# xeTaiz/vit-tf

Measured on AMD Instinct MI355X. Metric: slices/sec (ViT-S/8, 512^3 vol: feature volume + 16-query similarity), higher is better.
Workload: dtype fp16; 1 GPU; 512^3 CT-like synthetic volume (seed 0), ViT-S/8, fos 64: 1536 slices of 512x512 (N=4097) per step + 16-query similarity -> the metric's configuration (BASELINE configs[2]); engine_batch=512, weights=seeded synthetic vits8 (seed 0), parallelism=single GPU

## Files before the change

### vit-tf_amd/csrc/attention_pp64.hip

```cpp
#include "attn_common.h"

#include <stdlib.h>

namespace {

constexpr int NBUF = 3;
constexpr int QT = 256;
constexpr int KT = ATT_KT;
constexpr int KVB = ATT_KV_TILE_BYTES;
constexpr int BUFB = ATT_BUF_BYTES;

struct LdsBases { const char *ka0, *ka1, *ka2, *ka3, *va0, *va1; };
struct KFrag { s16x8_t k[4]; };
struct VFrag { s16x8_t v[4]; };
struct QFrag { s16x8_t q[4]; };
struct Blk {
  f32x16_t o0, o1, negm;
  float l_run;
};

__device__ __forceinline__ s16x8_t ld_k(const LdsBases& b, int i, int off) {
  const char* base = i == 0 ? b.ka0 : i == 1 ? b.ka1 : i == 2 ? b.ka2 : b.ka3;
  return *reinterpret_cast<const s16x8_t*>(base + off);
}
__device__ __forceinline__ s16x8_t ld_v(const LdsBases& b, int j, int off) {
  const int imm = off + 2048 * (j >> 1) + 512 * (j & 1);
  const s16x4_t lo = __builtin_amdgcn_ds_read_tr16_b64_v4i16((__attribute__((address_space(3))) s16x4_t*)(b.va0 + imm));
  const s16x4_t hi = __builtin_amdgcn_ds_read_tr16_b64_v4i16((__attribute__((address_space(3))) s16x4_t*)(b.va1 + imm + 1024));
  return __builtin_shufflevector(lo, hi, 0, 1, 2, 3, 4, 5, 6, 7);
}

template <int DT> __device__ __forceinline__ f32x16_t score_mfma(const KFrag& k, const QFrag& q, f32x16_t c) {
#pragma unroll
  for (int i = 0; i < 4; ++i) c = mfma32<DT>(k.k[i], q.q[i], c);
  return c;
}

__device__ __forceinline__ float tile_max(const f32x16_t& s) {
  float tmax = max3_f32(s[0], s[1], s[2]);
#pragma unroll
  for (int r = 3; r < 15; r += 2) tmax = max3_f32(tmax, s[r], s[r + 1]);
  tmax = fmaxf(tmax, s[15]);
  const unsigned tb = __float_as_uint(tmax);
  const auto sw = __builtin_amdgcn_permlane32_swap(tb, tb, false, false);
  return max3_f32(tmax, __uint_as_float(sw[0]), __uint_as_float(sw[1]));
}

__device__ unsigned g_rescales;

template <int DT> __device__ __forceinline__ constexpr float p_limit() { return DT == VITTF_FP16 ? 8192.f : 1073741824.f; }

template <int DT>
__device__ __forceinline__ float rescale_block(const LdsBases& b, Blk& X, const QFrag& qX, s16x8_t (&pX)[2], int ck_off, bool mask,
                                               int key0, int tokens, int h) {
  if ((threadIdx.x & 63) == 0) atomicAdd(&g_rescales, 1u);
  f32x16_t raw;
#pragma unroll
  for (int r = 0; r < 16; ++r) raw[r] = 0.f;
  KFrag kh;
#pragma unroll
  for (int i = 0; i < 4; ++i) kh.k[i] = ld_k(b, i, ck_off);
  raw = score_mfma<DT>(kh, qX, raw);
  if (mask) {
#pragma unroll
    for (int r = 0; r < 16; ++r)
      if (key0 + acc_row(r, h) >= tokens) raw[r] = -INFINITY;
  }
  const float tmax = tile_max(raw);
  const float delta = fmaxf(tmax + X.negm[0], 0.f);
  const float alpha = __builtin_amdgcn_exp2f(-delta);
  X.l_run *= alpha;
#pragma unroll
  for (int r = 0; r < 16; ++r) {
    X.o0[r] *= alpha;
    X.o1[r] *= alpha;
    X.negm[r] -= delta;
  }
  float psum0 = 0.f, psum1 = 0.f;
  u32x4_t u0, u1;
#pragma unroll
  for (int i = 0; i < 8; ++i) {
    const float e0 = __builtin_amdgcn_exp2f(raw[2 * i] + X.negm[2 * i]);
    const float e1 = __builtin_amdgcn_exp2f(raw[2 * i + 1] + X.negm[2 * i + 1]);
    psum0 += e0;
    psum1 += e1;
    const unsigned w = pack2_h16<DT>(e0, e1);
    if (i < 4) u0[i] = w; else u1[i - 4] = w;
  }
  pX[0] = __builtin_bit_cast(s16x8_t, u0);
  pX[1] = __builtin_bit_cast(s16x8_t, u1);
  return psum0 + psum1;
}

template <int DT, bool LOAD, bool MASK>
__device__ __forceinline__ void pp_phase(const LdsBases& b, Blk& X, const QFrag& qX, f32x16_t& sX, s16x8_t (&pX)[2], Blk& Y,
                                         const QFrag& qY, f32x16_t& sY, const s16x8_t (&pY)[2], KFrag& kf, VFrag& vf, int ck_off,
                                         int nk_off, int nv_off, int key0, int tokens, int h) {
  if constexpr (MASK) {
#pragma unroll
    for (int r = 0; r < 16; ++r)
      if (key0 + acc_row(r, h) >= tokens) sX[r] = -INFINITY;
  }
  float psum0 = 0.f, psum1 = 0.f;
  u32x4_t pk0, pk1;
#pragma unroll
  for (int g = 0; g < 8; ++g) {
    const int i = g & 3;
    if (g < 4) {
      sY = mfma32<DT>(kf.k[i], qY.q[i], i == 0 ? Y.negm : sY);
      if constexpr (LOAD) kf.k[i] = ld_k(b, i, nk_off);
    } else {
      if (i & 1) Y.o1 = mfma32<DT>(vf.v[i], pY[i >> 1], Y.o1);
      else       Y.o0 = mfma32<DT>(vf.v[i], pY[i >> 1], Y.o0);
      if constexpr (LOAD) vf.v[i] = ld_v(b, i, nv_off);
    }
    const float e0 = __builtin_amdgcn_exp2f(sX[2 * g]);
    const float e1 = __builtin_amdgcn_exp2f(sX[2 * g + 1]);
    if (g == 0) { psum0 = e0; psum1 = e1; } else { psum0 += e0; psum1 += e1; }
    const unsigned w = pack2_h16<DT>(e0, e1);
    if (g < 4) pk0[g] = w; else pk1[g - 4] = w;
    __builtin_amdgcn_sched_barrier(0);
  }
  float ps = psum0 + psum1;
  pX[0] = __builtin_bit_cast(s16x8_t, pk0);
  pX[1] = __builtin_bit_cast(s16x8_t, pk1);
  if (__builtin_expect(__any(!(ps <= p_limit<DT>())), 0)) ps = rescale_block<DT>(b, X, qX, pX, ck_off, MASK, key0, tokens, h);
  X.l_run += ps;
}

template <int DT>
__device__ __forceinline__ void pp_phase_rt(const LdsBases& b, Blk& X, const QFrag& qX, f32x16_t& sX, s16x8_t (&pX)[2], Blk& Y,
                                            const QFrag& qY, f32x16_t& sY, const s16x8_t (&pY)[2], KFrag& kf, VFrag& vf,
                                            int ck_off, int nk_off, int nv_off, bool do_s, bool do_o, bool load_k, bool load_v,
                                            bool mask, int key0, int tokens, int h) {
  if (do_s) sY = score_mfma<DT>(kf, qY, Y.negm);
  if (do_o) {
#pragma unroll
    for (int j = 0; j < 4; ++j) {
      if (j & 1) Y.o1 = mfma32<DT>(vf.v[j], pY[j >> 1], Y.o1);
      else       Y.o0 = mfma32<DT>(vf.v[j], pY[j >> 1], Y.o0);
    }
  }
  if (load_k) {
#pragma unroll
    for (int i = 0; i < 4; ++i) kf.k[i] = ld_k(b, i, nk_off);
  }
  if (load_v) {
#pragma unroll
    for (int j = 0; j < 4; ++j) vf.v[j] = ld_v(b, j, nv_off);
  }
  if (mask) {
#pragma unroll
    for (int r = 0; r < 16; ++r)
      if (key0 + acc_row(r, h) >= tokens) sX[r] = -INFINITY;
  }
  float psum0 = 0.f, psum1 = 0.f;
  u32x4_t pk0, pk1;
#pragma unroll
  for (int g = 0; g < 8; ++g) {
    const float e0 = __builtin_amdgcn_exp2f(sX[2 * g]);
    const float e1 = __builtin_amdgcn_exp2f(sX[2 * g + 1]);
    psum0 += e0;
    psum1 += e1;
    const unsigned w = pack2_h16<DT>(e0, e1);
    if (g < 4) pk0[g] = w; else pk1[g - 4] = w;
  }
  float ps = psum0 + psum1;
  pX[0] = __builtin_bit_cast(s16x8_t, pk0);
  pX[1] = __builtin_bit_cast(s16x8_t, pk1);
  if (__builtin_expect(__any(!(ps <= p_limit<DT>())), 0)) ps = rescale_block<DT>(b, X, qX, pX, ck_off, mask, key0, tokens, h);
  X.l_run += ps;
}

template <int DT>
__global__ __launch_bounds__(256, 2) void attn_pp64_kernel(const unsigned short* __restrict__ qkv, unsigned short* __restrict__ out,
                                                           int tokens, int heads, int q_tiles, int total) {
  __shared__ __attribute__((aligned(16))) char smem[NBUF * BUFB];
  const int tid = threadIdx.x;
  const int lane = tid & 63, wave = tid >> 6;
  const int h = lane >> 5, l31 = lane & 31;

  const int item = xcd_remap(blockIdx.x, total);
  const int qt = item % q_tiles;
  const int bh = item / q_tiles;
  const int hd = bh % heads, bi = bh / heads;
  const int dmodel = heads * 64;
  const int ld = 3 * dmodel;
  const unsigned short* base = qkv + (int64_t)bi * tokens * ld;

  const i32x4_t rsrc = lds_dma_rsrc(base, (unsigned)((int64_t)tokens * ld * 2));

  QFrag qa, qb;
  const int qrow_a = qt * QT + wave * 64 + l31, qrow_b = qrow_a + 32;
  {
    const unsigned short* pa_ = base + (int64_t)(qrow_a < tokens ? qrow_a : tokens - 1) * ld + hd * 64 + 8 * h;
    const unsigned short* pb_ = base + (int64_t)(qrow_b < tokens ? qrow_b : tokens - 1) * ld + hd * 64 + 8 * h;
#pragma unroll
    for (int i = 0; i < 4; ++i) {
      qa.q[i] = *reinterpret_cast<const s16x8_t*>(pa_ + 16 * i);
      qb.q[i] = *reinterpret_cast<const s16x8_t*>(pb_ + 16 * i);
    }
  }

  int voff_k, voff_v;
  {
    int r, cc, key, ch;
    tile_pos(tid, r, cc);
    voff_k = (r * ld + dmodel + hd * 64 + cc * 8) * 2;
    v_pos(tid, key, ch);
    voff_v = (key * ld + 2 * dmodel + hd * 64 + ch * 8) * 2;
  }
  const int tile_stride = KT * ld * 2, half_stride = 32 * ld * 2;
  const int nt = (tokens + KT - 1) / KT;
  const unsigned dma_dst = (unsigned)(size_t)LDS_PTR(smem) + (__builtin_amdgcn_readfirstlane(tid & ~63) << 4);
#define PP_STAGE_TILE(t_, bufi_)                                                                    \
  {                                                                                                 \
    const int so_ = (t_) * tile_stride;                                                             \
    const unsigned dst_ = dma_dst + (bufi_) * BUFB;                                                 \
    if ((t_) == nt - 1) {                                                                           \
      int vk_ = voff_k, vv_ = voff_v;    \
      asm volatile("" : "+v"(vk_), "+v"(vv_));                                                      \
      _Pragma("unroll") for (int i_ = 0; i_ < 2; ++i_) {                                            \
        lds_dma16(rsrc, dst_ + i_ * 4096, vk_ + so_ + i_ * half_stride, 0);                         \
        lds_dma16(rsrc, dst_ + KVB + i_ * 4096, vv_ + so_ + i_ * half_stride, 0);                   \
      }                                                                                             \
    } else {                                                                                        \
      _Pragma("unroll") for (int i_ = 0; i_ < 2; ++i_) {                                            \
        lds_dma16(rsrc, dst_ + i_ * 4096, voff_k, so_ + i_ * half_stride);                          \
        lds_dma16(rsrc, dst_ + KVB + i_ * 4096, voff_v, so_ + i_ * half_stride);                    \
      }                                                                                             \
    }                                                                                               \
  }

  LdsBases b;
  {
    const int p_l = l31 >> 1;
    const int bslot = (((l31 & 1) << 3) | h) ^ (p_l & 15);
    b.ka0 = smem + (p_l << 8) + ((bslot ^ 0) << 4);
    b.ka1 = smem + (p_l << 8) + ((bslot ^ 2) << 4);
    b.ka2 = smem + (p_l << 8) + ((bslot ^ 4) << 4);
    b.ka3 = smem + (p_l << 8) + ((bslot ^ 6) << 4);
    const int g16 = lane >> 4;
    const int tr_q = (lane & 15) >> 2;
    const int tr_p = lane & 3;
    const int tr_ch = 2 * (g16 & 1) + (tr_p >> 1);
    const int vl0 = 64 * (4 * h + tr_q) + 16 * (tr_ch ^ h) + 8 * (tr_p & 1);
    b.va0 = smem + vl0;
    b.va1 = smem + (vl0 ^ 32);
  }

  PP_STAGE_TILE(0, 0)
  if (nt > 1) PP_STAGE_TILE(1, 1)
  asm volatile("s_waitcnt vmcnt(0)" ::: "memory");
  __syncthreads();
  if (nt > 2) PP_STAGE_TILE(2, 2)
  asm volatile("" : "+v"(qa.q[0]), "+v"(qa.q[1]), "+v"(qa.q[2]), "+v"(qa.q[3]), "+v"(qb.q[0]), "+v"(qb.q[1]), "+v"(qb.q[2]), "+v"(qb.q[3]));

#define PP_TILE_BARRIER(BNEXT2)                                                                     \
  {                                                                                                 \
    asm volatile("s_waitcnt vmcnt(0)" ::: "memory");                                                \
    __syncthreads();                                                                                \
    if (t + 2 < nt) PP_STAGE_TILE(t + 2, BNEXT2)                                                    \
  }

  const bool active = __builtin_amdgcn_readfirstlane(qt * QT + wave * 64) < tokens;
  if (!active) {
    for (int t = 1; t < nt; ++t) {
      const int b2 = (t + 2) % NBUF;
      PP_TILE_BARRIER(b2)
    }
    return;
  }

  Blk A, B;
  f32x16_t sa, sb;
  s16x8_t pa[2], pb[2];
  KFrag kf;
  VFrag vf = {};
#pragma unroll
  for (int r = 0; r < 16; ++r) { A.o0[r] = 0.f; A.o1[r] = 0.f; A.negm[r] = 0.f; B.o0[r] = 0.f; B.o1[r] = 0.f; B.negm[r] = 0.f; }
  A.l_run = 0.f; B.l_run = 0.f;
  pa[0] = s16x8_t{}; pa[1] = s16x8_t{}; pb[0] = s16x8_t{}; pb[1] = s16x8_t{};
  {
#pragma unroll
    for (int i = 0; i < 4; ++i) kf.k[i] = ld_k(b, i, 0);
    sa = score_mfma<DT>(kf, qa, A.negm);
    sb = score_mfma<DT>(kf, qb, B.negm);
    if (nt == 1) {
#pragma unroll
      for (int r = 0; r < 16; ++r)
        if (acc_row(r, h) >= tokens) { sa[r] = -INFINITY; sb[r] = -INFINITY; }
    }
    const float ta = tile_max(sa), tb = tile_max(sb);
#pragma unroll
    for (int r = 0; r < 16; ++r) { A.negm[r] = -ta; sa[r] -= ta; B.negm[r] = -tb; sb[r] -= tb; }
  }

#define PP_TILE(RB_)                                                                                                        \
  {                                                                                                                         \
    constexpr int o_ = (RB_) * BUFB, on_ = (((RB_) + 1) % NBUF) * BUFB;                                                     \
    pp_phase<DT, true, false>(b, A, qa, sa, pa, B, qb, sb, pb, kf, vf, o_, o_ + 4096, o_ + KVB, 0, tokens, h);              \
    pp_phase<DT, false, false>(b, B, qb, sb, pb, A, qa, sa, pa, kf, vf, o_, 0, 0, 0, tokens, h);                            \
    pp_phase<DT, true, false>(b, A, qa, sa, pa, B, qb, sb, pb, kf, vf, o_ + 4096, on_, o_ + KVB + 4096, 0, tokens, h);      \
    pp_phase<DT, false, false>(b, B, qb, sb, pb, A, qa, sa, pa, kf, vf, o_ + 4096, 0, 0, 0, tokens, h);                     \
    ++t;                                                                                                                    \
  }
#define PP_COLD_TILE()                                                                                                      \
  {                                                                                                                         \
    const int o_ = (t % NBUF) * BUFB, on_ = ((t + 1) % NBUF) * BUFB;                                                        \
    const bool first_ = t == 0, last_ = t == nt - 1;                                                                        \
                      \
    const bool half_ = last_ && tokens - t * KT <= 32;                                                                      \
    int hc_ = h;             \
    asm volatile("" : "+v"(hc_));                                                                                           \
    pp_phase_rt<DT>(b, A, qa, sa, pa, B, qb, sb, pb, kf, vf, o_, o_ + 4096, o_ + KVB, !first_, !first_, !half_, true, last_, \
                    t * KT, tokens, hc_);                                                                                     \
    pp_phase_rt<DT>(b, B, qb, sb, pb, A, qa, sa, pa, kf, vf, o_, 0, 0, !half_, true, false, false, last_, t * KT, tokens, hc_); \
    if (!half_) {                                                                                                           \
      pp_phase_rt<DT>(b, A, qa, sa, pa, B, qb, sb, pb, kf, vf, o_ + 4096, on_, o_ + KVB + 4096, true, true, !last_, true,    \
                      last_, t * KT + 32, tokens, hc_);                                                                       \
      pp_phase_rt<DT>(b, B, qb, sb, pb, A, qa, sa, pa, kf, vf, o_ + 4096, 0, 0, !last_, true, false, false, last_,           \
                      t * KT + 32, tokens, hc_);                                                                              \
    }                                                                                                                       \
    ++t;                                                                                                                    \
  }
  int t = 0;
  PP_COLD_TILE()
  while (t + 3 <= nt - 1) {
    PP_TILE_BARRIER(0) PP_TILE(1)
    PP_TILE_BARRIER(1) PP_TILE(2)
    PP_TILE_BARRIER(2) PP_TILE(0)
  }
  while (t < nt) {
    const int b2_ = (t + 2) % NBUF;
    PP_TILE_BARRIER(b2_)
    PP_COLD_TILE()
  }
#undef PP_COLD_TILE
#undef PP_TILE
#undef PP_TILE_BARRIER
#undef PP_STAGE_TILE
#pragma unroll
  for (int j = 0; j < 4; ++j) {
    if (j & 1) B.o1 = mfma32<DT>(vf.v[j], pb[j >> 1], B.o1);
    else       B.o0 = mfma32<DT>(vf.v[j], pb[j >> 1], B.o0);
  }

  auto store = [&](const Blk& X, int qrow) {
    const unsigned lb = __float_as_uint(X.l_run);
    const auto sw = __builtin_amdgcn_permlane32_swap(lb, lb, false, false);
    const float inv = 1.0f / (__uint_as_float(sw[0]) + __uint_as_float(sw[1]));
    if (qrow < tokens) store_o_row<DT>(out + ((int64_t)bi * tokens + qrow) * dmodel + hd * 64, h, X.o0, X.o1, inv);
  };
  store(A, qrow_a);
  store(B, qrow_b);
}

}

extern "C" int64_t vittf_attention_rescale_count(int32_t reset) {
  unsigned v = 0;
  if (hipDeviceSynchronize() != hipSuccess) return VITTF_ERR_LAUNCH;
  if (hipMemcpyFromSymbol(&v, HIP_SYMBOL(g_rescales), sizeof(v)) != hipSuccess) return VITTF_ERR_LAUNCH;
  if (reset) {
    const unsigned z = 0;
    if (hipMemcpyToSymbol(HIP_SYMBOL(g_rescales), &z, sizeof(z)) != hipSuccess) return VITTF_ERR_LAUNCH;
  }
  return (int64_t)v;
}

int vittf_attention_pp64(const void* qkv, void* out, int32_t batch, int32_t tokens, int32_t heads, int32_t dtype, hipStream_t st) {
  const int q_tiles = (tokens + QT - 1) / QT;
  const int64_t total64 = (int64_t)batch * heads * q_tiles;
  if (total64 > (1 << 30)) return VITTF_ERR_INVALID_ARG;
  const int total = (int)total64;
  if (dtype == VITTF_BF16)
    hipLaunchKernelGGL((attn_pp64_kernel<VITTF_BF16>), dim3(total), dim3(256), 0, st, (const unsigned short*)qkv,
                       (unsigned short*)out, tokens, heads, q_tiles, total);
  else if (dtype == VITTF_FP16)
    hipLaunchKernelGGL((attn_pp64_kernel<VITTF_FP16>), dim3(total), dim3(256), 0, st, (const unsigned short*)qkv,
                       (unsigned short*)out, tokens, heads, q_tiles, total);
  else
    return VITTF_ERR_INVALID_ARG;
  return vittf_check_launch();
}
```

Before: 2374 slices/s.

## Fold CLS key into registers and add split-key path for ragged query tile

When the token count is 64k+1 (a CLS token plus a full patch grid), the CLS key/value is loaded into registers and folded into the softmax with dot2 instructions. The remaining keys then tile exactly, so the padded, masked final KV tile goes away. The last query tile, which holds at most 32 rows, gets a dedicated path: two waves split the keys between them and merge their partial softmax states through LDS, while the other two waves act as DMA producers. This adds code size and complexity, and a noinline call that may raise register pressure.

```diff
diff --git a/vit-tf_amd/csrc/attention_pp64.hip b/vit-tf_amd/csrc/attention_pp64.hip
--- a/vit-tf_amd/csrc/attention_pp64.hip
+++ b/vit-tf_amd/csrc/attention_pp64.hip
@@ -172,6 +172,218 @@
   X.l_run += ps;
 }
 
+
+struct ClsKV { s16x8_t k[4]; s16x8_t v[2]; };
+template <int DT> __device__ __forceinline__ ClsKV load_cls_kv(const unsigned short* base, int dmodel, int hd, int h, int l31) {
+  ClsKV c;
+  const unsigned short* pk_ = base + dmodel + hd * 64 + 8 * h;
+  const unsigned short* pv_ = base + 2 * dmodel + hd * 64 + l31;
+#pragma unroll
+  for (int i = 0; i < 4; ++i) c.k[i] = *reinterpret_cast<const s16x8_t*>(pk_ + 16 * i);
+#pragma unroll
+  for (int dv = 0; dv < 2; ++dv) {
+    c.v[dv] = s16x8_t{};
+    c.v[dv][0] = h == 0 ? (short)pv_[32 * dv] : (short)0;
+  }
+  return c;
+}
+template <int DT> __device__ __forceinline__ float dot2_h16(unsigned a, unsigned b, float c) {
+  if constexpr (DT == VITTF_BF16) return __builtin_amdgcn_fdot2_f32_bf16(__builtin_bit_cast(bf16x2_t, a), __builtin_bit_cast(bf16x2_t, b), c, false);
+  else return __builtin_amdgcn_fdot2(__builtin_bit_cast(f16x2_t, a), __builtin_bit_cast(f16x2_t, b), c, false);
+}
+template <int DT> __device__ __forceinline__ void cls_fold(const ClsKV& c, const QFrag& q, int h, float& tmax, Blk& X) {
+  typedef __attribute__((ext_vector_type(4))) unsigned u4_t;
+  float s0 = 0.f, s1 = 0.f;
+#pragma unroll
+  for (int i = 0; i < 4; ++i) {
+    const u4_t qu = __builtin_bit_cast(u4_t, q.q[i]), ku = __builtin_bit_cast(u4_t, c.k[i]);
+    s0 = dot2_h16<DT>(qu[0], ku[0], s0);
+    s1 = dot2_h16<DT>(qu[1], ku[1], s1);
+    s0 = dot2_h16<DT>(qu[2], ku[2], s0);
+    s1 = dot2_h16<DT>(qu[3], ku[3], s1);
+  }
+  const unsigned sb_ = __float_as_uint(s0 + s1);
+  const auto sw = __builtin_amdgcn_permlane32_swap(sb_, sb_, false, false);
+  const float sc = __uint_as_float(sw[0]) + __uint_as_float(sw[1]);
+  tmax = fmaxf(tmax, sc);
+  const float pc = __builtin_amdgcn_exp2f(sc - tmax);
+  X.l_run = h == 0 ? pc : 0.f;
+  u4_t pu = {0u, 0u, 0u, 0u};
+  pu[0] = h == 0 ? pack2_h16<DT>(pc, 0.f) : 0u;
+  const s16x8_t pf = __builtin_bit_cast(s16x8_t, pu);
+  X.o0 = mfma32<DT>(c.v[0], pf, X.o0);
+  X.o1 = mfma32<DT>(c.v[1], pf, X.o1);
+}
+
+struct RagCtx {
+  const unsigned short* base; unsigned short* orow;
+  int tokens, heads, hd, q0; unsigned lds0;
+};
+__device__ __forceinline__ unsigned uni(unsigned v) { return __builtin_amdgcn_readfirstlane(v); }
+template <typename T> __device__ __forceinline__ T* uni_ptr(T* p) {
+  const uint64_t v = reinterpret_cast<uint64_t>(p);
+  return reinterpret_cast<T*>(((uint64_t)uni((unsigned)(v >> 32)) << 32) | uni((unsigned)v));
+}
+
+template <int DT>
+__device__ __attribute__((noinline)) void run_ragged(RagCtx c) {
+  typedef __attribute__((address_space(3))) char lds_char;
+  typedef __attribute__((address_space(3))) float lds_float;
+  const unsigned short* const base = uni_ptr(c.base);
+  unsigned short* const orow = uni_ptr(c.orow);
+  const int tokens = (int)uni((unsigned)c.tokens), heads = (int)uni((unsigned)c.heads), hd = (int)uni((unsigned)c.hd);
+  const int q0 = (int)uni((unsigned)c.q0);
+  const unsigned lds0 = uni(c.lds0);
+  const int tid = threadIdx.x;
+  const int lane = tid & 63, wave = __builtin_amdgcn_readfirstlane(tid >> 6);
+  const int h = lane >> 5, l31 = lane & 31;
+  const int dmodel = heads * 64, ld = 3 * dmodel;
+  const bool cls = (tokens & (KT - 1)) == 1 && tokens > 1;
+  const int nt = cls ? (tokens - 1) / KT : (tokens + KT - 1) / KT;
+  const int mslot = (nt + 1) % NBUF;
+
+  if (wave >= 2) {
+    const i32x4_t rsrc = lds_dma_rsrc(base, (unsigned)((int64_t)tokens * ld * 2));
+    int vk[2], vv[2];
+#pragma unroll
+    for (int j = 0; j < 2; ++j) {
+      int r, cc, key, ch;
+      tile_pos(tid - 128 * j, r, cc);
+      vk[j] = ((r + (cls ? 1 : 0)) * ld + dmodel + hd * 64 + cc * 8) * 2;
+      v_pos(tid - 128 * j, key, ch);
+      vv[j] = ((key + (cls ? 1 : 0)) * ld + 2 * dmodel + hd * 64 + ch * 8) * 2;
+    }
+    const int tile_stride = KT * ld * 2, half_stride = 32 * ld * 2;
+    auto stage = [&](int t, int slot) {
+#pragma unroll
+      for (int j = 0; j < 2; ++j) {
+        const unsigned dst = lds0 + slot * BUFB + (wave - 2 * j) * 1024;
+#pragma unroll
+        for (int i = 0; i < 2; ++i) {
+          lds_dma16(rsrc, dst + i * 4096, vk[j] + t * tile_stride + i * half_stride, 0);
+          lds_dma16(rsrc, dst + KVB + i * 4096, vv[j] + t * tile_stride + i * half_stride, 0);
+        }
+      }
+    };
+    stage(0, 0);
+    if (nt > 1) stage(1, 1);
+    asm volatile("s_waitcnt vmcnt(0)" ::: "memory");
+    __syncthreads();
+    if (nt > 2) stage(2, 2);
+    for (int t = 1; t < nt; ++t) {
+      asm volatile("s_waitcnt vmcnt(0)" ::: "memory");
+      __syncthreads();
+      if (t + 2 < nt) stage(t + 2, (t + 2) % NBUF);
+    }
+    __syncthreads();
+    return;
+  }
+
+  QFrag qa;
+  const int qrow = q0 + l31;
+  {
+    const unsigned short* pa_ = base + (int64_t)(qrow < tokens ? qrow : tokens - 1) * ld + hd * 64 + 8 * h;
+#pragma unroll
+    for (int i = 0; i < 4; ++i) qa.q[i] = *reinterpret_cast<const s16x8_t*>(pa_ + 16 * i);
+  }
+  ClsKV ckv = {};
+  if (cls && wave == 0) ckv = load_cls_kv<DT>(base, dmodel, hd, h, l31);
+  LdsBases b;
+  {
+    const char* const smem = (const char*)(lds_char*)(size_t)lds0;
+    const int p_l = l31 >> 1;
+    const int bslot = (((l31 & 1) << 3) | h) ^ (p_l & 15);
+    b.ka0 = smem + (p_l << 8) + ((bslot ^ 0) << 4);
+    b.ka1 = smem + (p_l << 8) + ((bslot ^ 2) << 4);
+    b.ka2 = smem + (p_l << 8) + ((bslot ^ 4) << 4);
+    b.ka3 = smem + (p_l << 8) + ((bslot ^ 6) << 4);
+    const int g16 = lane >> 4;
+    const int tr_q = (lane & 15) >> 2;
+    const int tr_p = lane & 3;
+    const int tr_ch = 2 * (g16 & 1) + (tr_p >> 1);
+    const int vl0 = 64 * (4 * h + tr_q) + 16 * (tr_ch ^ h) + 8 * (tr_p & 1);
+    b.va0 = smem + vl0;
+    b.va1 = smem + (vl0 ^ 32);
+  }
+  Blk X;
+#pragma unroll
+  for (int r = 0; r < 16; ++r) { X.o0[r] = 0.f; X.o1[r] = 0.f; X.negm[r] = 0.f; }
+  X.l_run = 0.f;
+  const bool has_keys = cls || 32 * wave < tokens;
+  for (int t = 0; t < nt; ++t) {
+    __syncthreads();
+    if (!has_keys) continue;
+    const int ck = (t % NBUF) * BUFB + wave * 4096, cv = ck + KVB;
+    const int key0 = t * KT + 32 * wave;
+    const bool mask = !cls && t == nt - 1;
+    KFrag kf;
+    VFrag vf;
+#pragma unroll
+    for (int i = 0; i < 4; ++i) kf.k[i] = ld_k(b, i, ck);
+#pragma unroll
+    for (int j = 0; j < 4; ++j) vf.v[j] = ld_v(b, j, cv);
+    f32x16_t s = score_mfma<DT>(kf, qa, X.negm);
+    if (mask) {
+#pragma unroll
+      for (int r = 0; r < 16; ++r)
+        if (key0 + acc_row(r, h) >= tokens) s[r] = -INFINITY;
+    }
+    if (t == 0) {
+      float tm = tile_max(s);
+      if (cls && wave == 0) cls_fold<DT>(ckv, qa, h, tm, X);
+#pragma unroll
+      for (int r = 0; r < 16; ++r) { X.negm[r] = -tm; s[r] -= tm; }
+    }
+    float psum0 = 0.f, psum1 = 0.f;
+    u32x4_t pk0, pk1;
+#pragma unroll
+    for (int g = 0; g < 8; ++g) {
+      const float e0 = __builtin_amdgcn_exp2f(s[2 * g]);
+      const float e1 = __builtin_amdgcn_exp2f(s[2 * g + 1]);
+      psum0 += e0;
+      psum1 += e1;
+      const unsigned w = pack2_h16<DT>(e0, e1);
+      if (g < 4) pk0[g] = w; else pk1[g - 4] = w;
+    }
+    float ps = psum0 + psum1;
+    s16x8_t pX[2];
+    pX[0] = __builtin_bit_cast(s16x8_t, pk0);
+    pX[1] = __builtin_bit_cast(s16x8_t, pk1);
+    if (__builtin_expect(__any(!(ps <= p_limit<DT>())), 0)) ps = rescale_block<DT>(b, X, qa, pX, ck, mask, key0, tokens, h);
+    X.l_run += ps;
+#pragma unroll
+    for (int j = 0; j < 4; ++j) {
+      if (j & 1) X.o1 = mfma32<DT>(vf.v[j], pX[j >> 1], X.o1);
+      else       X.o0 = mfma32<DT>(vf.v[j], pX[j >> 1], X.o0);
+    }
+  }
+
+  lds_float* const mrg = (lds_float*)(size_t)(lds0 + mslot * BUFB) + lane;
+  if (wave == 1) {
+    mrg[0] = has_keys ? -X.negm[0] : -INFINITY;
+    mrg[64] = X.l_run;
+#pragma unroll
+    for (int r = 0; r < 16; ++r) { mrg[64 * (2 + r)] = X.o0[r]; mrg[64 * (18 + r)] = X.o1[r]; }
+  }
+  __syncthreads();
+  if (wave == 1) return;
+  {
+    const float m0 = -X.negm[0], m1 = mrg[0];
+    const float m = fmaxf(m0, m1);
+    const float a0 = __builtin_amdgcn_exp2f(m0 - m), a1 = __builtin_amdgcn_exp2f(m1 - m);
+    X.l_run = X.l_run * a0 + mrg[64] * a1;
+#pragma unroll
+    for (int r = 0; r < 16; ++r) {
+      X.o0[r] = X.o0[r] * a0 + mrg[64 * (2 + r)] * a1;
+      X.o1[r] = X.o1[r] * a0 + mrg[64 * (18 + r)] * a1;
+    }
+    const unsigned lb = __float_as_uint(X.l_run);
+    const auto sw = __builtin_amdgcn_permlane32_swap(lb, lb, false, false);
+    const float inv = 1.0f / (__uint_as_float(sw[0]) + __uint_as_float(sw[1]));
+    if (qrow < tokens) store_o_row<DT>(orow + (int64_t)qrow * dmodel, h, X.o0, X.o1, inv);
+  }
+}
+
 template <int DT>
 __global__ __launch_bounds__(256, 2) void attn_pp64_kernel(const unsigned short* __restrict__ qkv, unsigned short* __restrict__ out,
                                                            int tokens, int heads, int q_tiles, int total) {
@@ -188,6 +400,11 @@
   const int ld = 3 * dmodel;
   const unsigned short* base = qkv + (int64_t)bi * tokens * ld;
 
+  if (qt == q_tiles - 1 && tokens - qt * QT <= 32) {
+    run_ragged<DT>(RagCtx{base, out + (int64_t)bi * tokens * dmodel + hd * 64, tokens, heads, hd, qt * QT, (unsigned)(size_t)LDS_PTR(smem)});
+    return;
+  }
+
   const i32x4_t rsrc = lds_dma_rsrc(base, (unsigned)((int64_t)tokens * ld * 2));
 
   QFrag qa, qb;
@@ -201,6 +418,9 @@
       qb.q[i] = *reinterpret_cast<const s16x8_t*>(pb_ + 16 * i);
     }
   }
+  const bool cls = (tokens & (KT - 1)) == 1 && tokens > 1;
+  ClsKV ckv = {};
+  if (cls) ckv = load_cls_kv<DT>(base, dmodel, hd, h, l31);
 
   int voff_k, voff_v;
   {
@@ -209,15 +429,18 @@
     voff_k = (r * ld + dmodel + hd * 64 + cc * 8) * 2;
     v_pos(tid, key, ch);
     voff_v = (key * ld + 2 * dmodel + hd * 64 + ch * 8) * 2;
+    if (cls) { voff_k += ld * 2; voff_v += ld * 2; }
   }
   const int tile_stride = KT * ld * 2, half_stride = 32 * ld * 2;
-  const int nt = (tokens + KT - 1) / KT;
+  const int nt = cls ? (tokens - 1) / KT : (tokens + KT - 1) / KT;
+  const int t_rag = cls ? -1 : nt - 1;
+  const int t_hot_end = cls ? nt : nt - 1;
   const unsigned dma_dst = (unsigned)(size_t)LDS_PTR(smem) + (__builtin_amdgcn_readfirstlane(tid & ~63) << 4);
 #define PP_STAGE_TILE(t_, bufi_)                                                                    \
   {                                                                                                 \
     const int so_ = (t_) * tile_stride;                                                             \
     const unsigned dst_ = dma_dst + (bufi_) * BUFB;                                                 \
-    if ((t_) == nt - 1) {                                                                           \
+    if ((t_) == t_rag) {                                                                            \
       int vk_ = voff_k, vv_ = voff_v;    \
       asm volatile("" : "+v"(vk_), "+v"(vv_));                                                      \
       _Pragma("unroll") for (int i_ = 0; i_ < 2; ++i_) {                                            \
@@ -286,12 +509,16 @@
     for (int i = 0; i < 4; ++i) kf.k[i] = ld_k(b, i, 0);
     sa = score_mfma<DT>(kf, qa, A.negm);
     sb = score_mfma<DT>(kf, qb, B.negm);
-    if (nt == 1) {
+    if (nt == 1 && !cls) {
 #pragma unroll
       for (int r = 0; r < 16; ++r)
         if (acc_row(r, h) >= tokens) { sa[r] = -INFINITY; sb[r] = -INFINITY; }
     }
-    const float ta = tile_max(sa), tb = tile_max(sb);
+    float ta = tile_max(sa), tb = tile_max(sb);
+    if (cls) {
+      cls_fold<DT>(ckv, qa, h, ta, A);
+      cls_fold<DT>(ckv, qb, h, tb, B);
+    }
 #pragma unroll
     for (int r = 0; r < 16; ++r) { A.negm[r] = -ta; sa[r] -= ta; B.negm[r] = -tb; sb[r] -= tb; }
   }
@@ -308,25 +535,25 @@
 #define PP_COLD_TILE()                                                                                                      \
   {                                                                                                                         \
     const int o_ = (t % NBUF) * BUFB, on_ = ((t + 1) % NBUF) * BUFB;                                                        \
-    const bool first_ = t == 0, last_ = t == nt - 1;                                                                        \
+    const bool first_ = t == 0, last_ = t == nt - 1, mask_ = last_ && !cls;                                                 \
                       \
     const bool half_ = last_ && tokens - t * KT <= 32;                                                                      \
     int hc_ = h;             \
     asm volatile("" : "+v"(hc_));                                                                                           \
-    pp_phase_rt<DT>(b, A, qa, sa, pa, B, qb, sb, pb, kf, vf, o_, o_ + 4096, o_ + KVB, !first_, !first_, !half_, true, last_, \
+    pp_phase_rt<DT>(b, A, qa, sa, pa, B, qb, sb, pb, kf, vf, o_, o_ + 4096, o_ + KVB, !first_, !first_, !half_, true, mask_, \
                     t * KT, tokens, hc_);                                                                                     \
-    pp_phase_rt<DT>(b, B, qb, sb, pb, A, qa, sa, pa, kf, vf, o_, 0, 0, !half_, true, false, false, last_, t * KT, tokens, hc_); \
+    pp_phase_rt<DT>(b, B, qb, sb, pb, A, qa, sa, pa, kf, vf, o_, 0, 0, !half_, true, false, false, mask_, t * KT, tokens, hc_); \
     if (!half_) {                                                                                                           \
       pp_phase_rt<DT>(b, A, qa, sa, pa, B, qb, sb, pb, kf, vf, o_ + 4096, on_, o_ + KVB + 4096, true, true, !last_, true,    \
-                      last_, t * KT + 32, tokens, hc_);                                                                       \
-      pp_phase_rt<DT>(b, B, qb, sb, pb, A, qa, sa, pa, kf, vf, o_ + 4096, 0, 0, !last_, true, false, false, last_,           \
+                      mask_, t * KT + 32, tokens, hc_);                                                                       \
+      pp_phase_rt<DT>(b, B, qb, sb, pb, A, qa, sa, pa, kf, vf, o_ + 4096, 0, 0, !last_, true, false, false, mask_,           \
                       t * KT + 32, tokens, hc_);                                                                              \
     }                                                                                                                       \
     ++t;                                                                                                                    \
   }
   int t = 0;
   PP_COLD_TILE()
-  while (t + 3 <= nt - 1) {
+  while (t + 3 <= t_hot_end) {
     PP_TILE_BARRIER(0) PP_TILE(1)
     PP_TILE_BARRIER(1) PP_TILE(2)
     PP_TILE_BARRIER(2) PP_TILE(0)
```

After: 2395 slices/s, median of 6. No clear change (+0.9%).

## Split keys across waves for tiny tail query tiles and merge partial softmax in LDS

Applied to the files above, without the earlier changes.

With N=4097 and QT=256, the last query tile holds a single row, so only one of its four waves does work while it still streams every KV tile. For tail tiles with at most 32 rows, each wave now processes every fourth KV tile for the same query rows. The partial outputs, maxima and sums are then merged through the LDS ring using a log-sum-exp combine. This removes the serial critical path of the tail block. In exchange it adds a merge step and a second code path with its own masking and rescale logic.

```diff
diff --git a/vit-tf_amd/csrc/attention_pp64.hip b/vit-tf_amd/csrc/attention_pp64.hip
--- a/vit-tf_amd/csrc/attention_pp64.hip
+++ b/vit-tf_amd/csrc/attention_pp64.hip
@@ -172,6 +172,54 @@
   X.l_run += ps;
 }
 
+constexpr int KS_ROWS = 32;
+constexpr int KS_STRIDE = 34 * 64;
+static_assert(4 * KS_STRIDE * 4 <= NBUF * BUFB, "the key split merges through the ring");
+
+template <int DT>
+__device__ __forceinline__ void ks_half(const LdsBases& b, Blk& X, const QFrag& q, int k_off, int v_off, bool first, bool mask,
+                                        int key0, int tokens, int h) {
+  KFrag kf;
+  VFrag vf;
+#pragma unroll
+  for (int i = 0; i < 4; ++i) kf.k[i] = ld_k(b, i, k_off);
+#pragma unroll
+  for (int j = 0; j < 4; ++j) vf.v[j] = ld_v(b, j, v_off);
+  f32x16_t s = score_mfma<DT>(kf, q, X.negm);
+  if (mask) {
+#pragma unroll
+    for (int r = 0; r < 16; ++r)
+      if (key0 + acc_row(r, h) >= tokens) s[r] = -INFINITY;
+  }
+  if (first) {
+    const float tm = tile_max(s);
+#pragma unroll
+    for (int r = 0; r < 16; ++r) { X.negm[r] = -tm; s[r] -= tm; }
+  }
+  float psum0 = 0.f, psum1 = 0.f;
+  u32x4_t pk0, pk1;
+#pragma unroll
+  for (int g = 0; g < 8; ++g) {
+    const float e0 = __builtin_amdgcn_exp2f(s[2 * g]);
+    const float e1 = __builtin_amdgcn_exp2f(s[2 * g + 1]);
+    psum0 += e0;
+    psum1 += e1;
+    const unsigned w = pack2_h16<DT>(e0, e1);
+    if (g < 4) pk0[g] = w; else pk1[g - 4] = w;
+  }
+  float ps = psum0 + psum1;
+  s16x8_t p[2];
+  p[0] = __builtin_bit_cast(s16x8_t, pk0);
+  p[1] = __builtin_bit_cast(s16x8_t, pk1);
+  if (__builtin_expect(__any(!(ps <= p_limit<DT>())), 0)) ps = rescale_block<DT>(b, X, q, p, k_off, mask, key0, tokens, h);
+  X.l_run += ps;
+#pragma unroll
+  for (int j = 0; j < 4; ++j) {
+    if (j & 1) X.o1 = mfma32<DT>(vf.v[j], p[j >> 1], X.o1);
+    else       X.o0 = mfma32<DT>(vf.v[j], p[j >> 1], X.o0);
+  }
+}
+
 template <int DT>
 __global__ __launch_bounds__(256, 2) void attn_pp64_kernel(const unsigned short* __restrict__ qkv, unsigned short* __restrict__ out,
                                                            int tokens, int heads, int q_tiles, int total) {
@@ -190,8 +238,9 @@
 
   const i32x4_t rsrc = lds_dma_rsrc(base, (unsigned)((int64_t)tokens * ld * 2));
 
+  const bool ksplit = qt >= 1 && tokens - qt * QT <= KS_ROWS;
   QFrag qa, qb;
-  const int qrow_a = qt * QT + wave * 64 + l31, qrow_b = qrow_a + 32;
+  const int qrow_a = qt * QT + (ksplit ? 0 : wave * 64) + l31, qrow_b = ksplit ? qrow_a : qrow_a + 32;
   {
     const unsigned short* pa_ = base + (int64_t)(qrow_a < tokens ? qrow_a : tokens - 1) * ld + hd * 64 + 8 * h;
     const unsigned short* pb_ = base + (int64_t)(qrow_b < tokens ? qrow_b : tokens - 1) * ld + hd * 64 + 8 * h;
@@ -263,6 +312,60 @@
     if (t + 2 < nt) PP_STAGE_TILE(t + 2, BNEXT2)                                                    \
   }
 
+  if (ksplit) {
+    const int wv = __builtin_amdgcn_readfirstlane(wave);
+    Blk A;
+#pragma unroll
+    for (int r = 0; r < 16; ++r) { A.o0[r] = 0.f; A.o1[r] = 0.f; A.negm[r] = 0.f; }
+    A.l_run = 0.f;
+    bool first = true;
+    for (int t = 0; t < nt; ++t) {
+      if (t > 0) {
+        const int b2 = (t + 2) % NBUF;
+        PP_TILE_BARRIER(b2)
+      }
+      if ((t & 3) != wv) continue;
+      const int o_ = (t % NBUF) * BUFB;
+      const bool last_ = t == nt - 1;
+      int hc_ = h;
+      asm volatile("" : "+v"(hc_));
+      ks_half<DT>(b, A, qa, o_, o_ + KVB, first, last_, t * KT, tokens, hc_);
+      first = false;
+      if (!(last_ && tokens - t * KT <= 32))
+        ks_half<DT>(b, A, qa, o_ + 4096, o_ + KVB + 4096, false, last_, t * KT + 32, tokens, hc_);
+    }
+    __syncthreads();
+    float* mrg = reinterpret_cast<float*>(smem);
+    {
+      float* mw = mrg + wv * KS_STRIDE + lane;
+#pragma unroll
+      for (int r = 0; r < 16; ++r) { mw[r * 64] = A.o0[r]; mw[(16 + r) * 64] = A.o1[r]; }
+      mw[32 * 64] = A.negm[0];
+      mw[33 * 64] = A.l_run;
+    }
+    __syncthreads();
+    if (wv != 0) return;
+    float negm = mrg[32 * 64 + lane];
+#pragma unroll
+    for (int w = 1; w < 4; ++w) negm = fminf(negm, mrg[w * KS_STRIDE + 32 * 64 + lane]);
+    float l = 0.f;
+#pragma unroll
+    for (int r = 0; r < 16; ++r) { A.o0[r] = 0.f; A.o1[r] = 0.f; }
+#pragma unroll
+    for (int w = 0; w < 4; ++w) {
+      const float* mw = mrg + w * KS_STRIDE + lane;
+      const float alpha = __builtin_amdgcn_exp2f(negm - mw[32 * 64]);
+      l += mw[33 * 64] * alpha;
+#pragma unroll
+      for (int r = 0; r < 16; ++r) { A.o0[r] += mw[r * 64] * alpha; A.o1[r] += mw[(16 + r) * 64] * alpha; }
+    }
+    const unsigned lb = __float_as_uint(l);
+    const auto sw = __builtin_amdgcn_permlane32_swap(lb, lb, false, false);
+    const float inv = 1.0f / (__uint_as_float(sw[0]) + __uint_as_float(sw[1]));
+    if (qrow_a < tokens) store_o_row<DT>(out + ((int64_t)bi * tokens + qrow_a) * dmodel + hd * 64, h, A.o0, A.o1, inv);
+    return;
+  }
+
   const bool active = __builtin_amdgcn_readfirstlane(qt * QT + wave * 64) < tokens;
   if (!active) {
     for (int t = 1; t < nt; ++t) {
```

New measurement: 2234 slices/s before, 2243 slices/s after, median of 6. No clear change (+0.4%).
